# xander683/ConstructionScenePoseEstimation

Measured on AMD Instinct MI355X. Metric: annotated frames/sec (RGB+seg+2D kpts) at 1920×1080, 1/2/4/8 MI355X, higher is better.
Workload: dtype f32

## Files before the change

constructionsceneposeestimation_amd/build.py:

```python
from __future__ import annotations

import os
import shutil
import subprocess
import sys

PKG = os.path.dirname(os.path.abspath(__file__))
ROOT = os.path.dirname(PKG)
LIB = os.path.join(PKG, "libcsg.so")
SOURCES = [os.path.join(PKG, "csrc", "csg_kernels.hip"), os.path.join(PKG, "csrc", "csg_encode.hip"),
           os.path.join(PKG, "csrc", "csg_crops.hip"), os.path.join(PKG, "csrc", "csg_spans.hip"),
           os.path.join(PKG, "csrc", "csg_points.hip"), os.path.join(PKG, "csrc", "csg_amodal_spans.hip"),
           os.path.join(PKG, "csrc", "csg_mask_png.hip"), os.path.join(PKG, "csrc", "csg_jpeg.hip"),
           os.path.join(PKG, "csrc", "csg_voxels.hip"), os.path.join(PKG, "csrc", "csg_sensor.hip"),
           os.path.join(PKG, "csrc", "csg_fps.hip"),
           os.path.join(PKG, "csrc", "csg_api.cpp"), os.path.join(PKG, "csrc", "csg_passes.cpp")]
DEPS = SOURCES + [os.path.join(PKG, "csrc", "csg_ctx.h"), os.path.join(PKG, "csrc", "csg_kernels.h"), os.path.join(PKG, "csrc", "csg_encode.h"),
                  os.path.join(PKG, "csrc", "csg_deflate.h"), os.path.join(PKG, "csrc", "csg_widen.h"),
                  os.path.join(PKG, "csrc", "csg_crops.h"), os.path.join(PKG, "csrc", "csg_spans.h"),
                  os.path.join(PKG, "csrc", "csg_points.h"),
                  os.path.join(PKG, "csrc", "csg_amodal_spans.h"), os.path.join(PKG, "csrc", "csg_raster_math.h"),
                  os.path.join(PKG, "csrc", "csg_amodal_tri.inc"),
                  os.path.join(PKG, "csrc", "csg_alpha_box.h"),
                  os.path.join(PKG, "csrc", "csg_mask_png.h"), os.path.join(PKG, "csrc", "csg_bitio.h"),
                  os.path.join(PKG, "csrc", "csg_jpeg.h"), os.path.join(PKG, "csrc", "csg_voxels.h"),
                  os.path.join(PKG, "csrc", "csg_sensor.h"), os.path.join(PKG, "csrc", "csg_fps.h"),
                  os.path.join(ROOT, "include", "csg_api.h")]
ARCH = os.environ.get("CSG_OFFLOAD_ARCH", "gfx950")
IO_LIB = os.path.join(PKG, "libcsgio.so")
IO_SOURCES = [os.path.join(PKG, "csrc", "csg_io.cpp")]
IO_DEPS = IO_SOURCES + [os.path.join(ROOT, "include", "csg_io.h"), os.path.join(PKG, "csrc", "csg_repr.h")]
IO_FLAGS = ["-O3", "-std=c++17", "-fPIC", "-shared", "-Wall", "-pthread"]
JSON_EXT = os.path.join(PKG, "_csgjson.so")
JSON_SOURCES = [os.path.join(PKG, "csrc", "csg_json.cpp"), os.path.join(PKG, "csrc", "csg_repr.h")]

FLAGS = ["-O3", "-std=c++17", "-fPIC", "-shared", "-ffp-contract=off", f"--offload-arch={ARCH}", "-Wall", "-pthread"]


def hipcc() -> str:
    for c in (os.environ.get("HIPCC"), "/opt/rocm/bin/hipcc", shutil.which("hipcc")):
        if c and os.path.exists(c):
            return c
    raise RuntimeError("hipcc not found (ROCm required to build libcsg.so)")


def needs_build(lib: str = LIB, deps=None) -> bool:
    deps = DEPS if deps is None else deps
    if not os.path.exists(lib):
        return True
    t = os.path.getmtime(lib)
    return any(os.path.getmtime(p) > t for p in deps)


def build(force: bool = False, verbose: bool = False) -> str:
    if force or needs_build():
        cmd = [hipcc(), *FLAGS, "-o", LIB + ".tmp", *SOURCES]
        if verbose:
            print(" ".join(cmd), file=sys.stderr)
        subprocess.run(cmd, check=True)
        os.replace(LIB + ".tmp", LIB)
    return LIB


def build_io(force: bool = False, verbose: bool = False) -> str:
    if force or needs_build(IO_LIB, IO_DEPS):
        cxx = os.environ.get("CXX") or shutil.which("g++") or "g++"
        cmd = [cxx, *IO_FLAGS, "-o", IO_LIB + ".tmp", *IO_SOURCES, "-lz"]
        if verbose:
            print(" ".join(cmd), file=sys.stderr)
        subprocess.run(cmd, check=True)
        os.replace(IO_LIB + ".tmp", IO_LIB)
    return IO_LIB


def build_json(force: bool = False, verbose: bool = False) -> str:
    if force or needs_build(JSON_EXT, JSON_SOURCES):
        import sysconfig
        cxx = os.environ.get("CXX") or shutil.which("g++") or "g++"
        cmd = [cxx, "-O2", "-std=c++17", "-fPIC", "-shared", "-Wall", f"-I{sysconfig.get_paths()['include']}", "-o",
               JSON_EXT + ".tmp", JSON_SOURCES[0]]
        if verbose:
            print(" ".join(cmd), file=sys.stderr)
        subprocess.run(cmd, check=True)
        os.replace(JSON_EXT + ".tmp", JSON_EXT)
    return JSON_EXT


if __name__ == "__main__":
    print(build(force="--force" in sys.argv, verbose=True))
    print(build_io(force="--force" in sys.argv, verbose=True))
    print(build_json(force="--force" in sys.argv, verbose=True))
```

constructionsceneposeestimation_amd/csrc/csg_kernels.hip:

```cpp
#include <math.h>

#include <algorithm>

#include <type_traits>

#include "csg_crops.h"
#include "csg_kernels.h"
#include "csg_raster_math.h"

namespace csg {

#ifndef CSG_ABLATION
#define CSG_ABLATION 0
#endif
#define DBG(d) (CSG_ABLATION ? (d) : 0u)

constexpr uint64_t kEmptyKey = ~0ull;

__device__ __forceinline__ uint32_t fbits(float f) { return __float_as_uint(f); }

template <int Ctrl, int RowMask, int BankMask>
__device__ __forceinline__ uint32_t dpp_add(uint32_t v) {
  return v + (uint32_t)__builtin_amdgcn_update_dpp(0, (int)v, Ctrl, RowMask, BankMask, false);
}
__device__ __forceinline__ uint32_t wave_incl_scan(uint32_t v) {
  v = dpp_add<0x111, 0xf, 0xf>(v);
  v = dpp_add<0x112, 0xf, 0xf>(v);
  v = dpp_add<0x114, 0xf, 0xf>(v);
  v = dpp_add<0x118, 0xf, 0xf>(v);
  v = dpp_add<0x142, 0xa, 0xf>(v);
  v = dpp_add<0x143, 0xc, 0xf>(v);
  return v;
}

template <bool kTrail = true, int NB = kBlock>
__device__ __forceinline__ uint32_t block_excl_scan(uint32_t v, uint32_t* wsum, uint32_t& total) {
  const uint32_t inc = wave_incl_scan(v);
  const int w = threadIdx.x >> 6, lane = threadIdx.x & 63;
  if (lane == 63) wsum[w] = inc;
  __syncthreads();
  uint32_t off = 0, tot = 0;
#pragma unroll
  for (int k = 0; k < NB / 64; ++k) {
    const uint32_t x = wsum[k];
    off += (k < w) ? x : 0u;
    tot += x;
  }
  if (kTrail) __syncthreads();
  total = tot;
  return off + inc - v;
}

__device__ __forceinline__ void frame_camera(const float* V, const float* P, float* cam) {
#pragma unroll
  for (int i = 0; i < 3; ++i) {
#pragma unroll
    for (int j = 0; j < 3; ++j) cam[i * 3 + j] = V[j * 4 + i];
    cam[9 + i] = -((V[0 * 4 + i] * V[3] + V[1 * 4 + i] * V[7]) + V[2 * 4 + i] * V[11]);
  }
  cam[12] = P[0];
  cam[13] = -P[5];
  cam[14] = -P[2];
  cam[15] = -P[6];
}

__device__ __forceinline__ void unproject(const float* cam, int px, int py, float d, float out[3]) {
  const float a = ((float)px + 0.5f) - cam[14], bq = ((float)py + 0.5f) - cam[15];
  const float xc = (a * d) / cam[12], yc = -((bq * d) / cam[13]), zc = -d;
#pragma unroll
  for (int i = 0; i < 3; ++i) out[i] = ((cam[i * 3 + 0] * xc + cam[i * 3 + 1] * yc) + cam[i * 3 + 2] * zc) + cam[9 + i];
}

__device__ __forceinline__ uint32_t half_bits(float x) {
  const _Float16 h = (_Float16)(x + 0.0f);
  return (uint32_t)__builtin_bit_cast(uint16_t, h);
}

__global__ __launch_bounds__(256) void k_clip(SceneDev s, BatchDev b) {
  const uint32_t f = blockIdx.y;
  const uint32_t i = blockIdx.x * blockDim.x + threadIdx.x;
  const FrameDev& fr = b.frames[f];
  const uint32_t raw = fr.xform_set;
  const uint32_t set = raw < b.n_sets ? raw : 0u;
  if (i < s.n_inst) {
    const float* M = b.models + ((size_t)set * s.n_inst + i) * 16;
    float m[16], vm[16], c[16];
#pragma unroll
    for (int k = 0; k < 16; ++k) m[k] = M[k];
    mat4_mul(fr.view, m, vm);
    mat4_mul(fr.proj, vm, c);
    float* o = b.clip + ((size_t)f * s.n_inst + i) * 12;
#pragma unroll
    for (int k = 0; k < 4; ++k) {
      o[k] = c[k];
      o[4 + k] = c[4 + k];
      o[8 + k] = c[12 + k];
    }
  }
  if (blockIdx.x == 0 && threadIdx.x == 0) {
    b.fset[f] = set;
    if (raw >= b.n_sets) atomicOr(b.overflow, kOvBadSet);
    float pv[16];
    mat4_mul(fr.proj, fr.view, pv);
    float* o = b.pv + (size_t)f * 12;
    for (int k = 0; k < 4; ++k) {
      o[k] = pv[k];
      o[4 + k] = pv[4 + k];
      o[8 + k] = pv[12 + k];
    }
    frame_camera(fr.view, fr.proj, b.cam + (size_t)f * kCamFloats);
  }
}

__device__ __forceinline__ uint32_t rec_tile_rect(const SubRec& r, uint32_t ys) {
  const uint32_t px0 = r.g1.z & 0xFFFFu, py0 = r.g1.z >> 16, px1 = r.g1.w & 0xFFFFu, py1 = r.g1.w >> 16;
  return (px0 / kTileW) | (((py0 / kTileH) >> ys) << 8) | ((px1 / kTileW) << 16) | (((py1 / kTileH) >> ys) << 24);
}

__device__ __forceinline__ uint32_t rect_ty0(uint32_t rc, uint32_t ys) { return ((rc >> 8) & 255u) << ys; }
__device__ __forceinline__ uint32_t rect_ty1(uint32_t rc, uint32_t ys, uint32_t tiles_y) {
  return min((((rc >> 24) + 1u) << ys) - 1u, tiles_y - 1u);
}

__device__ __forceinline__ uint32_t rect_area(uint32_t rc, uint32_t ys, uint32_t tiles_y) {
  const uint32_t tx0 = rc & 255u, tx1 = (rc >> 16) & 255u;
  return (tx1 - tx0 + 1) * (rect_ty1(rc, ys, tiles_y) - rect_ty0(rc, ys) + 1);
}


__device__ __forceinline__ uint32_t rect_tile(uint32_t rc, uint32_t q, uint32_t tiles_x, uint32_t ys) {
  const uint32_t tx0 = rc & 255u, ty0 = rect_ty0(rc, ys), tx1 = (rc >> 16) & 255u;
  const uint32_t w = tx1 - tx0 + 1;
  const uint32_t r = small_div(q, w);
  return __umul24(ty0 + r, tiles_x) + tx0 + (q - __umul24(r, w));
}

typedef uint32_t v4u32 __attribute__((ext_vector_type(4)));

__device__ __forceinline__ void setup_chunk(const SceneDev& s, const BatchDev& b, const Chunk& ch, uint32_t f,
                                            int tid, int lane, uint4* sw);

__global__ __launch_bounds__(256) __attribute__((amdgpu_waves_per_eu(8, 8))) void k_setup(
    SceneDev s, BatchDev b, const Chunk* __restrict__ chunks, uint32_t n_chunks) {
  const uint32_t f = blockIdx.x, chunk = blockIdx.y + blockIdx.z * gridDim.y;
  if (chunk >= n_chunks) return;
  const int tid = threadIdx.x, lane = tid & 63;
  if (DBG(b.dbg) & 32u) return;
  const Chunk& ch = chunks[chunk];
  {
    const CullOut o = corner_out(s, ch, b.clip + ((size_t)f * s.n_inst + ch.inst) * 12, lane & 7);
    const uint64_t m8 = 0xFFull;
    const bool cull = ((__ballot(o.n) & m8) == m8) || ((__ballot(o.f) & m8) == m8) ||
                      ((__ballot(o.l) & m8) == m8) || ((__ballot(o.r) & m8) == m8) ||
                      ((__ballot(o.t) & m8) == m8) || ((__ballot(o.b) & m8) == m8);
    if (cull || (DBG(b.dbg) & 64u)) return;
  }
  static_assert(16 * kRecGroups <= 2 * 64, "two chunk stores per lane");
  __shared__ uint4 tstage[kBlock / 64][16 * kRecGroups];
  setup_chunk(s, b, ch, f, tid, lane, tstage[tid >> 6]);
}

__device__ __forceinline__ void setup_chunk(const SceneDev& s, const BatchDev& b, const Chunk& ch, uint32_t f,
                                            int tid, int lane, uint4* sw) {
  const uint32_t i = ch.inst;
  const float* Cm = b.clip + ((size_t)f * s.n_inst + i) * 12;

  SubRec r0, r1;
  uint4 c2 = make_uint4(0u, 0u, 0u, 0u), c3 = c2, c4 = c2;
  int nrec = 0;
  if ((uint32_t)tid < ch.count) {
    const uint32_t g = ch.soup + tid;
    Cv3 v[3];
    float c[12];
#pragma unroll
    for (int k = 0; k < 12; ++k) c[k] = Cm[k];
    const float* tp = s.tri_pos + (size_t)g * 9;
#pragma unroll
    for (int k = 0; k < 3; ++k) {
      const float px = tp[3 * k], py = tp[3 * k + 1], pz = tp[3 * k + 2];
      v[k].x = dot4(c + 0, px, py, pz);
      v[k].y = dot4(c + 4, px, py, pz);
      v[k].w = dot4(c + 8, px, py, pz);
    }
    const float nearc = s.near_clip, farc = s.far_clip;
    const float Wf = (float)s.W, Hf = (float)s.H;
    bool on = true, of = true, ol = true, orr = true, ot = true, ob = true;
#pragma unroll
    for (int k = 0; k < 3; ++k) {
      on &= v[k].w < nearc;
      of &= v[k].w > farc;
      ol &= v[k].x < 0.0f;
      orr &= v[k].x > Wf * v[k].w;
      ot &= v[k].y < 0.0f;
      ob &= v[k].y > Hf * v[k].w;
    }
    if ((DBG(b.dbg) & 0x10000u) && !(on | of | ol | orr | ot | ob)) {
      if (v[0].x == 1.2345e-30f && b.inst) b.inst[0] = 1;
    } else if (!(on | of | ol | orr | ot | ob)) {
      const uint32_t uid = (i << s.uid_shift) | g;
      Cv3 q0 = v[0], q1 = v[1], q2 = v[2], q3 = v[2];
      int nq = 3;
      const bool in0 = v[0].w >= nearc, in1 = v[1].w >= nearc, in2 = v[2].w >= nearc;
      if (!(in0 && in1 && in2)) {
        auto cross_pt = [&](const Cv3& a, const Cv3& bb) {
          const float tt = (nearc - a.w) / (bb.w - a.w);
          Cv3 rr;
          rr.x = a.x + tt * (bb.x - a.x);
          rr.y = a.y + tt * (bb.y - a.y);
          rr.w = nearc;
          return rr;
        };
        auto sel = [](bool c, const Cv3& a, const Cv3& bb) {
          Cv3 rr;
          rr.x = c ? a.x : bb.x;
          rr.y = c ? a.y : bb.y;
          rr.w = c ? a.w : bb.w;
          return rr;
        };
        const Cv3 I01 = cross_pt(v[0], v[1]), I12 = cross_pt(v[1], v[2]), I20 = cross_pt(v[2], v[0]);
        const int code = (int)in0 | ((int)in1 << 1) | ((int)in2 << 2);
        q0 = sel(code == 2 || code == 6, I01, sel(code == 4, I12, v[0]));
        q1 = sel(code == 1 || code == 5, I01, sel(code == 4, v[2], v[1]));
        q2 = sel(code == 1 || code == 4, I20, sel(code == 6, v[2], I12));
        q3 = sel(code == 3 || code == 6, I20, v[2]);
        nq = (code == 1 || code == 2 || code == 4) ? 3 : 4;
      }
      auto emit_tri_r = [&](const Cv3& a, float ra, const Cv3& bb, float rb, const Cv3& cc, float rc) {
        float su[3], sv[3];
        su[0] = a.x * ra; sv[0] = a.y * ra;
        su[1] = bb.x * rb; sv[1] = bb.y * rb;
        su[2] = cc.x * rc; sv[2] = cc.y * rc;
        SubRec rr;
        if (make_rec(s, su, sv, rr)) {
          if (nrec == 0) r0 = rr; else r1 = rr;
          ++nrec;
        }
      };
      auto emit_tri = [&](const Cv3& a, const Cv3& bb, const Cv3& cc) {
        emit_tri_r(a, rcp_w(a.w), bb, rcp_w(bb.w), cc, rcp_w(cc.w));
      };
      if (nq >= 3) emit_tri(q0, q1, q2);
      if (nq >= 4) emit_tri(q0, q2, q3);
      if (nrec > 0) {
        Hom h;
        hom_setup(v, h);
        if (!h.ok) {
          nrec = 0;
        } else {
          const InstSetDev is = b.iset[(size_t)b.fset[f] * s.n_inst + i];
          const uint32_t atex = is.atex == kNoAlpha ? kNoAlpha : rec_atex(is.atex, is.athr), atex_wh = is.atex_wh;
          if (is.atex != kNoAlpha && is.athr >= 255u) nrec = 0;
          float D[3], U[3] = {0.0f, 0.0f, 0.0f}, V[3] = {0.0f, 0.0f, 0.0f};
          depth_plane(h.A, h.B, h.C, h.invdet, D);
          if (is.alpha_uv) {
            const float* tu = s.tri_uv + (size_t)g * 6;
            float uv[6];
#pragma unroll
            for (int k = 0; k < 6; ++k) uv[k] = tu[k];
            uv_planes(h.A, h.B, h.C, h.invdet, uv, U, V);
            if (is.trim && nq == 3 && in0 && in1 && in2 && nrec == 1) {
              const float4 bx = s.tri_abox[g];
              const bool none = bx.x > bx.y;
              const float B = none ? 0.0f : fmaxf(fmaxf(fabsf(bx.x), fabsf(bx.y)), fmaxf(fabsf(bx.z), fabsf(bx.w)));
              float m;
              if (B < INFINITY &&
                  alpha_trim_guard(v, uv, U, V, D, (float)max(atex_wh & 0xFFFFu, atex_wh >> 16), B, m)) {
                int px0 = (int)(r0.g1.z & 0xFFFFu), py0 = (int)(r0.g1.z >> 16);
                int px1 = (int)(r0.g1.w & 0xFFFFu), py1 = (int)(r0.g1.w >> 16);
                if (none || !alpha_trim_box(U, V, D, bx, m, px0, py0, px1, py1)) {
                  nrec = 0;
                } else {
                  r0.g1.z = (uint32_t)px0 | ((uint32_t)py0 << 16);
                  r0.g1.w = (uint32_t)px1 | ((uint32_t)py1 << 16);
                }
              }
            }
          }
          c2 = make_uint4(uid, atex, __float_as_uint(D[0]), __float_as_uint(D[1]));
          c3 = make_uint4(__float_as_uint(U[0]), __float_as_uint(V[0]), __float_as_uint(U[1]), __float_as_uint(V[1]));
          c4 = make_uint4(__float_as_uint(U[2]), __float_as_uint(V[2]), __float_as_uint(D[2]), atex_wh);
        }
      }
    }
  }
  const uint64_t b1 = __ballot(nrec >= 1), b2 = __ballot(nrec >= 2);
  const uint64_t lt = (lane == 0) ? 0ull : (~0ull >> (64 - lane));
  const uint32_t mine = (uint32_t)(__popcll(b1 & lt) + __popcll(b2 & lt));
  const uint32_t wtot = (uint32_t)(__popcll(b1) + __popcll(b2));
  uint32_t wbase = 0;
  if (lane == 0 && wtot) wbase = atomicAdd(&b.rec_count[f * kCounterStride], wtot);
  wbase = __shfl(wbase, 0, 64);
  if (DBG(b.dbg) & 128u) {
    if (nrec == 3 && b.inst) b.inst[0] = r0.g0.x + r1.g0.x + c2.x + c3.x + c4.x;
    return;
  }
  const uint64_t rbase = b.slab[f].rec_base;
  const uint32_t rcap = b.slab[f].rec_cap;
  if (lane == 0 && wbase + wtot > rcap) atomicOr(b.overflow, 1u);
  uint4* dst = reinterpret_cast<uint4*>(b.recs + rbase);
  const size_t lim = (size_t)rcap * kRecGroups;
  auto put = [&](uint32_t at, const SubRec& r) {
    uint4* o = sw + at * kRecGroups;
    o[0] = r.g0;
    o[1] = r.g1;
    o[2] = c2;
    o[3] = c3;
    o[4] = c4;
  };
  for (uint32_t p0 = 0; p0 < wtot; p0 += 16) {
    if (nrec > 0 && mine - p0 < 16u) put(mine - p0, r0);
    if (nrec > 1 && mine + 1u - p0 < 16u) put(mine + 1u - p0, r1);
    __builtin_amdgcn_fence(__ATOMIC_SEQ_CST, "wavefront");
    __builtin_amdgcn_wave_barrier();
    const uint32_t nch = min(16u, wtot - p0) * kRecGroups;
    const size_t at = ((size_t)wbase + p0) * kRecGroups;
#pragma unroll
    for (uint32_t c = (uint32_t)lane; c < 2u * 64u; c += 64u)
      if (c < nch && at + c < lim) {
        const uint4 q = sw[c];
        const v4u32 w = {q.x, q.y, q.z, q.w};
        __builtin_nontemporal_store(w, reinterpret_cast<v4u32*>(dst + at + c));
      }
    __builtin_amdgcn_fence(__ATOMIC_SEQ_CST, "wavefront");
    __builtin_amdgcn_wave_barrier();
  }
  if (nrec > 0 && wbase + mine < rcap) b.rect[rbase + wbase + mine] = rec_tile_rect(r0, s.rect_ys);
  if (nrec > 1 && wbase + mine + 1 < rcap) b.rect[rbase + wbase + mine + 1] = rec_tile_rect(r1, s.rect_ys);
}

constexpr int kBinRpt = 4;
constexpr uint32_t kBinRound = kBlock * kBinRpt;
constexpr uint32_t kBinBand = 32768;

__device__ __forceinline__ int find_bin_item(const uint32_t* pre, uint32_t j) {
  int lo = 0;
#pragma unroll
  for (int step = 256; step > 0; step >>= 2) {
    const uint32_t a = pre[lo + step], b2 = pre[lo + 2 * step], c = pre[lo + 3 * step];
    lo += ((a <= j) + (b2 <= j) + (c <= j)) * step;
  }
  return lo;
}

constexpr uint32_t kCountDirect = 4;
template <uint32_t kDirect, typename Single>
__device__ __forceinline__ uint32_t bin_round_setup(const uint32_t* rect, uint32_t base, uint32_t n, uint32_t* lrc,
                                                    uint32_t* pre, uint32_t* wsum, const SceneDev& s, Single single) {
  const int tid = threadIdx.x;
  const uint32_t r0 = base + (uint32_t)tid * kBinRpt;
  uint32_t rc[kBinRpt], area[kBinRpt], sum = 0;
  static_assert(kBinRpt == 4, "one 16-B rect load per thread");
  uint4 v = make_uint4(0u, 0u, 0u, 0u);
  if (r0 + 3 < n) {
    v = *reinterpret_cast<const uint4*>(rect + r0);
  } else {
    if (r0 < n) v.x = rect[r0];
    if (r0 + 1 < n) v.y = rect[r0 + 1];
    if (r0 + 2 < n) v.z = rect[r0 + 2];
  }
  rc[0] = v.x; rc[1] = v.y; rc[2] = v.z; rc[3] = v.w;
#pragma unroll
  for (int q = 0; q < kBinRpt; ++q) {
    area[q] = (r0 + (uint32_t)q < n) ? rect_area(rc[q], s.rect_ys, s.tiles_y) : 0u;
    lrc[tid * kBinRpt + q] = rc[q];
    if (kDirect && area[q] && area[q] <= kDirect) {
#pragma clang loop unroll(disable)
      for (uint32_t a = 0; a < area[q]; ++a) single(q, rect_tile(rc[q], a, s.tiles_x, s.rect_ys));
      area[q] = 0u;
    }
  }
#pragma unroll
  for (int q = 0; q < kBinRpt; ++q) sum += area[q];
  uint32_t total;
  uint32_t ex = block_excl_scan(sum, wsum, total);
#pragma unroll
  for (int q = 0; q < kBinRpt; ++q) {
    pre[tid * kBinRpt + q] = ex;
    ex += area[q];
  }
  if (tid == kBlock - 1) pre[kBinRound] = ex;
  return total;
}

template <bool kBanded>
__global__ __launch_bounds__(256) void k_count(SceneDev s, BatchDev b) {
  extern __shared__ __attribute__((aligned(16))) uint32_t dyn_count[];
  const uint32_t band = min(s.n_tiles, kBinBand);
  uint32_t* hist = dyn_count;
  uint32_t* pre = dyn_count + ((band + 3u) & ~3u);
  uint32_t* lrc = pre + kBinRound + 4;
  uint32_t* wsum = lrc + kBinRound;
  const uint32_t f = blockIdx.y;
  const int tid = threadIdx.x;
  const uint32_t n = min(b.rec_count[f * kCounterStride], b.slab[f].rec_cap);
  const uint32_t* rect = b.rect + b.slab[f].rec_base;
  uint32_t* bc = b.bcount + ((size_t)f * gridDim.x + blockIdx.x) * s.n_tiles;
  for (uint32_t t0 = 0; t0 < s.n_tiles; t0 += band) {
    const uint32_t nb = min(band, s.n_tiles - t0);
    for (uint32_t t = tid; t < nb; t += kBlock) hist[t] = 0;
    __syncthreads();
    for (uint32_t base = blockIdx.x * kBinRound; base < n; base += gridDim.x * kBinRound) {
      const uint32_t total = bin_round_setup<kCountDirect>(rect, base, n, lrc, pre, wsum, s,
                                                   [&](int, uint32_t t) {
                                                     if (!kBanded || t - t0 < nb) atomicAdd(&hist[t - t0], 1u);
                                                   });
      __syncthreads();
      for (uint32_t j = tid; j < total; j += kBlock) {
        const int k = find_bin_item(pre, j);
        const uint32_t t = rect_tile(lrc[k], j - pre[k], s.tiles_x, s.rect_ys);
        if (!kBanded || t - t0 < nb) atomicAdd(&hist[t - t0], 1u);
      }
      __syncthreads();
    }
    for (uint32_t t = tid; t < nb; t += kBlock) bc[t0 + t] = hist[t];
    __syncthreads();
  }
}

__global__ __launch_bounds__(256) void k_colscan(SceneDev s, BatchDev b) {
  const uint32_t f = blockIdx.y, t = blockIdx.x * kBlock + threadIdx.x;
  if (t >= s.n_tiles) return;
  uint32_t* col = b.bcount + (size_t)f * b.bin_blocks * s.n_tiles + t;
  uint32_t run = 0;
#pragma unroll 8
  for (uint32_t k = 0; k < b.bin_blocks; ++k) {
    const uint32_t v = col[(size_t)k * s.n_tiles];
    col[(size_t)k * s.n_tiles] = run;
    run += v;
  }
  b.tile_count[(size_t)f * s.n_tiles + t] = run;
}

__device__ __forceinline__ uint64_t wave_incl_scan64(uint64_t v, int lane) {
#pragma unroll
  for (int o = 1; o < 64; o <<= 1) {
    const uint64_t t = __shfl_up(v, o, 64);
    if (lane >= o) v += t;
  }
  return v;
}

__global__ __launch_bounds__(64) void k_plan(const FrameDev* __restrict__ frames, uint32_t F, uint32_t def_rec,
                                             uint32_t def_bin, uint64_t rec_pool, uint64_t bin_pool, int use_hints,
                                             Slab* __restrict__ slab, uint64_t* __restrict__ need) {
  const int lane = threadIdx.x;
  uint64_t cr = 0, cb = 0;
  for (uint32_t f0 = 0; f0 < F; f0 += 64) {
    const uint32_t f = f0 + (uint32_t)lane;
    uint32_t rc = 0, bc = 0;
    if (f < F) {
      const uint32_t rh = use_hints ? frames[f].records_hint : 0u, bh = use_hints ? frames[f].bins_hint : 0u;
      rc = rh ? ((min(rh, 0x7FFFFFF0u) + 3u) & ~3u) : def_rec;
      bc = bh ? ((min(bh, 0x7FFFFFF0u) + 3u) & ~3u) : def_bin;
    }
    const uint64_t ir = wave_incl_scan64(rc, lane), ib = wave_incl_scan64(bc, lane);
    if (f < F) {
      Slab sl;
      sl.rec_base = min(cr + ir - rc, rec_pool);
      sl.bin_base = min(cb + ib - bc, bin_pool);
      sl.rec_cap = (uint32_t)min((uint64_t)rc, rec_pool - sl.rec_base);
      sl.bin_cap = (uint32_t)min((uint64_t)bc, bin_pool - sl.bin_base);
      sl.pad[0] = sl.pad[1] = 0u;
      slab[f] = sl;
    }
    cr += __shfl(ir, 63, 64);
    cb += __shfl(ib, 63, 64);
  }
  if (lane == 0) {
    need[0] = max(need[0], cr);
    need[1] = max(need[1], cb);
  }
}

__global__ __launch_bounds__(256) void k_scan(SceneDev s, BatchDev b) {
  __shared__ uint32_t wsum[kBlock / 64];
  __shared__ uint32_t carry;
  const uint32_t f = blockIdx.x;
  const uint32_t* tc = b.tile_count + (size_t)f * s.n_tiles;
  uint32_t* to = b.tile_off + (size_t)f * (s.n_tiles + 1);
  if (threadIdx.x == 0) carry = 0;
  __syncthreads();
  for (uint32_t base = 0; base < s.n_tiles; base += kBlock) {
    const uint32_t t = base + threadIdx.x;
    const uint32_t v = t < s.n_tiles ? tc[t] : 0u;
    uint32_t tot;
    const uint32_t ex = block_excl_scan(v, wsum, tot);
    const uint32_t c0 = carry;
    if (t < s.n_tiles) to[t] = c0 + ex;
    __syncthreads();
    if (threadIdx.x == 0) carry = c0 + tot;
    __syncthreads();
  }
  if (threadIdx.x == 0) {
    to[s.n_tiles] = carry;
    if (carry > b.slab[f].bin_cap) atomicOr(b.overflow, 2u);
  }
}

template <bool kBanded>
__global__ __launch_bounds__(256) void k_bin(SceneDev s, BatchDev b) {
  extern __shared__ uint32_t dyn[];
  uint32_t* hist = dyn;
  __shared__ uint32_t pre[kBinRound + 1];
  __shared__ uint32_t lrc[kBinRound];
  __shared__ uint32_t wsum[kBlock / 64];
  const uint32_t f = blockIdx.y;
  const int tid = threadIdx.x;
  const Slab sb = b.slab[f];
  const uint32_t n = min(b.rec_count[f * kCounterStride], sb.rec_cap);
  const uint32_t* rect = b.rect + sb.rec_base;
  const uint32_t* toff = b.tile_off + (size_t)f * (s.n_tiles + 1);
  uint32_t* bins = b.bins + sb.bin_base;
  const uint32_t* bo = b.bcount + ((size_t)f * gridDim.x + blockIdx.x) * s.n_tiles;
  const uint32_t* tcnt = b.tile_count + (size_t)f * s.n_tiles;
  const uint32_t band = min(s.n_tiles, kBinBand);
  for (uint32_t t0 = 0; t0 < s.n_tiles; t0 += band) {
    const uint32_t nb = min(band, s.n_tiles - t0);
    for (uint32_t t = tid; t < nb; t += kBlock)
      hist[t] = toff[t0 + t] + tcnt[t0 + t] - bo[t0 + t] - 1u;
    __syncthreads();
    for (uint32_t base = blockIdx.x * kBinRound; base < n; base += gridDim.x * kBinRound) {
      const uint32_t total = bin_round_setup<0>(rect, base, n, lrc, pre, wsum, s, [](int, uint32_t) {});
      __syncthreads();
      for (uint32_t j = tid; j < total; j += kBlock) {
        const int k = find_bin_item(pre, j);
        const uint32_t t = rect_tile(lrc[k], j - pre[k], s.tiles_x, s.rect_ys);
        if (!kBanded || t - t0 < nb) {
          const uint32_t slot = atomicSub(&hist[t - t0], 1u);
          if (slot < sb.bin_cap) bins[slot] = base + (uint32_t)k;
        }
      }
      __syncthreads();
    }
  }
}

template <bool Small>
__device__ __forceinline__ void row_span(const uint4& g0, const uint4& g1, int ox, int oy, int ly, int x0, int x1,
                                         int& xl, int& xr, bool no_exact) {
  using T = typename std::conditional<Small, int32_t, int64_t>::type;
  const int32_t RX[3] = {(int32_t)g0.x, (int32_t)g0.y, (int32_t)g0.z};
  const int32_t RY[3] = {(int32_t)g0.w, (int32_t)g1.x, (int32_t)g1.y};
  const int32_t OX = ox * 256, OY = oy * 256;
  const int32_t cy = ly * 256 + 128;
  T c0[3];
  int32_t dys[3];
  float lo = -1.0e30f, hi = 1.0e30f;
  const int ea[3] = {1, 2, 0}, eb[3] = {2, 0, 1};
#pragma unroll
  for (int e = 0; e < 3; ++e) {
    const int32_t ax = RX[ea[e]] - OX, ay = RY[ea[e]] - OY;
    const int32_t dx = RX[eb[e]] - RX[ea[e]];
    const int32_t dy = RY[eb[e]] - RY[ea[e]];
    const int bias = (dy < 0 || (dy == 0 && dx > 0)) ? 0 : -1;
    if constexpr (Small) c0[e] = __mul24(dx, cy - ay) + __mul24(dy, ax) + bias;
    else c0[e] = (int64_t)dx * (cy - ay) + (int64_t)dy * ax + bias;
    dys[e] = dy;
    const float t = (float)c0[e] * __builtin_amdgcn_rcpf((float)dy);
    hi = (dy > 0) ? fminf(hi, t) : hi;
    lo = (dy < 0) ? fmaxf(lo, t) : lo;
    hi = (dy == 0 && c0[e] < 0) ? -1.0e30f : hi;
  }
  constexpr float kEps = 1.0f / 64.0f;
  const float lc = (lo - 128.0f) * (1.0f / 256.0f), hc = (hi - 128.0f) * (1.0f / 256.0f);
  const float lcc = fminf(fmaxf(lc, (float)x0 - 1.0f), (float)x1 + 1.0f);
  const float hcc = fmaxf(fminf(hc, (float)x1 + 1.0f), (float)x0 - 1.0f);
  xl = max((int)ceilf(lcc - kEps), x0);
  xr = min((int)floorf(hcc + kEps), x1);
  const float fl = lcc - floorf(lcc), fh = hcc - floorf(hcc);
  const bool walk_l = lc > (float)x0 - 0.5f && lc < (float)x1 + 0.5f && (fl <= kEps || fl >= 1.0f - kEps);
  const bool walk_r = hc > (float)x0 - 0.5f && hc < (float)x1 + 0.5f && (fh <= kEps || fh >= 1.0f - kEps);
  if (no_exact) return;
  auto covers = [&](int lx) {
    const int32_t cx = lx * 256 + 128;
    bool in = true;
#pragma unroll
    for (int e = 0; e < 3; ++e) {
      if constexpr (Small) in &= c0[e] - __mul24(dys[e], cx) >= 0;
// ... 1531 lines not shown
```

constructionsceneposeestimation_amd/csrc/csg_raster_math.h:

```cpp
#pragma once
#include <math.h>

#include "csg_kernels.h"

namespace csg {

constexpr int kSmallCover = 4;
constexpr float kGuardPx = 1048576.0f;

typedef float f32x2 __attribute__((ext_vector_type(2)));

__device__ __forceinline__ float dot4(const float* r, float x, float y, float z) {
  return ((r[0] * x + r[1] * y) + r[2] * z) + r[3];
}

__device__ __forceinline__ void mat4_mul(const float* a, const float* b, float* c) {
#pragma unroll
  for (int i = 0; i < 4; ++i)
#pragma unroll
    for (int j = 0; j < 4; ++j)
      c[i * 4 + j] = ((a[i * 4 + 0] * b[0 * 4 + j] + a[i * 4 + 1] * b[1 * 4 + j]) + a[i * 4 + 2] * b[2 * 4 + j]) +
                     a[i * 4 + 3] * b[3 * 4 + j];
}

#ifndef CSG_FAST_RCP
#define CSG_FAST_RCP 1
#endif
__device__ __forceinline__ float rcp_ieee(float x) {
#if CSG_FAST_RCP
  const float r0 = __builtin_amdgcn_rcpf(x);
  const float e = __builtin_fmaf(-x, r0, 1.0f);
  return __builtin_fmaf(e, r0, r0);
#else
  return 1.0f / x;
#endif
}

struct Cv3 { float x, y, w; };

struct Hom {
  float A[3], B[3], C[3];
  float invdet;
  bool ok;
};

__device__ __forceinline__ void hom_setup(const Cv3* v, Hom& h) {
  const int ea[3] = {1, 2, 0}, eb[3] = {2, 0, 1};
#pragma unroll
  for (int k = 0; k < 3; ++k) {
    const Cv3 a = v[ea[k]], b = v[eb[k]];
    h.A[k] = a.y * b.w - a.w * b.y;
    h.B[k] = a.w * b.x - a.x * b.w;
    h.C[k] = a.x * b.y - a.y * b.x;
  }
  const float det = (v[0].x * h.A[0] + v[0].y * h.B[0]) + v[0].w * h.C[0];
  h.ok = det != 0.0f;
  const float ad = fabsf(det);
  h.invdet = !h.ok ? 0.0f : (ad >= 0x1p-126f && ad <= 0x1p126f) ? rcp_ieee(det) : 1.0f / det;
}

__device__ __forceinline__ void depth_plane(const float* A, const float* B, const float* C, float invdet, float* D) {
  D[0] = ((A[0] + A[1]) + A[2]) * invdet;
  D[1] = ((B[0] + B[1]) + B[2]) * invdet;
  D[2] = ((C[0] + C[1]) + C[2]) * invdet;
}
__device__ __forceinline__ void uv_planes(const float* A, const float* B, const float* C, float invdet,
                                          const float* uv, float* U, float* V) {
  U[0] = ((A[0] * uv[0] + A[1] * uv[2]) + A[2] * uv[4]) * invdet;
  U[1] = ((B[0] * uv[0] + B[1] * uv[2]) + B[2] * uv[4]) * invdet;
  U[2] = ((C[0] * uv[0] + C[1] * uv[2]) + C[2] * uv[4]) * invdet;
  V[0] = ((A[0] * uv[1] + A[1] * uv[3]) + A[2] * uv[5]) * invdet;
  V[1] = ((B[0] * uv[1] + B[1] * uv[3]) + B[2] * uv[5]) * invdet;
  V[2] = ((C[0] * uv[1] + C[1] * uv[3]) + C[2] * uv[5]) * invdet;
}

__device__ __forceinline__ float plane_at(float p0, float p1, float p2, float fx, float fy) {
  return (p0 * fx + p1 * fy) + p2;
}

struct TexTap { uint32_t i00, i10, i01, i11; int wx, wy; };

__device__ __forceinline__ int wrap_index(float fu, int n) {
  const float nf = (float)n;
  if (fu >= 0.0f && fu < nf) return (int)fu;
  const float q = floorf(fu * __builtin_amdgcn_rcpf(nf));
  float r = fu - q * nf;
  r += r < 0.0f ? nf : 0.0f;
  r -= r >= nf ? nf : 0.0f;
  return (int)r;
}

__device__ __forceinline__ f32x2 texel_coords(float u, float v, int tw, int th) {
  const f32x2 a = {u, 1.0f - v}, n = {(float)tw, (float)th};
  return a * n - 0.5f;
}

__device__ __forceinline__ TexTap tex_taps(int tw, int th, float u, float v) {
  const f32x2 t2 = texel_coords(u, v, tw, th);
  float tu = t2.x, tv = t2.y;
  if (!(fabsf(tu) < 8388608.0f)) tu = 0.0f;
  if (!(fabsf(tv) < 8388608.0f)) tv = 0.0f;
  const float fu = floorf(tu), fv = floorf(tv);
  TexTap t;
  t.wx = (int)((tu - fu) * 256.0f) & 255;
  t.wy = (int)((tv - fv) * 256.0f) & 255;
  tw &= 0x7FFF;
  const int x0 = wrap_index(fu, tw) & 0x3FFF, y0 = wrap_index(fv, th) & 0x3FFF;
  const int x1 = (x0 + 1 == tw) ? 0 : x0 + 1;
  const int y1 = (y0 + 1 == th) ? 0 : y0 + 1;
  const uint32_t r0 = __umul24((uint32_t)y0, (uint32_t)tw), r1 = __umul24((uint32_t)y1, (uint32_t)tw);
  t.i00 = r0 + (uint32_t)x0; t.i10 = r0 + (uint32_t)x1;
  t.i01 = r1 + (uint32_t)x0; t.i11 = r1 + (uint32_t)x1;
  return t;
}

__device__ __forceinline__ int bilerp8(uint32_t c00, uint32_t c10, uint32_t c01, uint32_t c11, int wx, int wy) {
  const uint32_t ax = 256u - (uint32_t)wx, ay = 256u - (uint32_t)wy;
  const uint32_t top = __umul24(c00, ax) + __umul24(c10, (uint32_t)wx);
  const uint32_t bot = __umul24(c01, ax) + __umul24(c11, (uint32_t)wx);
  return (int)((__umul24(top, ay) + __umul24(bot, (uint32_t)wy) + 32768u) >> 16);
}

__device__ __forceinline__ int div255(uint32_t x) { return (int)(__umul24(x, 32897u) >> 23); }

__device__ __forceinline__ int tex_channel(uint32_t c00, uint32_t c10, uint32_t c01, uint32_t c11, int sh, int wx,
                                           int wy) {
  return bilerp8((c00 >> sh) & 255u, (c10 >> sh) & 255u, (c01 >> sh) & 255u, (c11 >> sh) & 255u, wx, wy);
}

__device__ __forceinline__ void tex_sample(const SceneDev& s, int tid, float u, float v, int out[4]) {
  const TexDesc t = s.texd[tid];
  const TexTap k = tex_taps((int)t.width, (int)t.height, u, v);
  const uint32_t* base = reinterpret_cast<const uint32_t*>(s.texels) + t.offset;
  const uint32_t c00 = base[k.i00], c10 = base[k.i10], c01 = base[k.i01], c11 = base[k.i11];
#pragma unroll
  for (int c = 0; c < 4; ++c) out[c] = tex_channel(c00, c10, c01, c11, 8 * c, k.wx, k.wy);
}

__device__ __forceinline__ bool alpha_pass(const uint32_t* aquad, const uint32_t* acls, uint32_t offset, uint32_t wh,
                                           int thr, float u, float v) {
  const int tw = (int)(wh & 0xFFFFu), th = (int)(wh >> 16);
  const f32x2 t2 = texel_coords(u, v, tw, th);
  float tu = t2.x, tv = t2.y;
  if (!(fabsf(tu) < 8388608.0f)) tu = 0.0f;
  if (!(fabsf(tv) < 8388608.0f)) tv = 0.0f;
  const float fu = floorf(tu), fv = floorf(tv);
  const uint32_t idx = offset + __umul24((uint32_t)wrap_index(fv, th) & 0x3FFFu, (uint32_t)tw & 0x7FFFu) +
                       ((uint32_t)wrap_index(fu, tw) & 0x3FFFu);
  const uint32_t cl = (acls[idx >> 4] >> (2u * (idx & 15u))) & 3u;
  if (cl != 3u) return cl != 0u;
  const int wx = (int)((tu - fu) * 256.0f) & 255, wy = (int)((tv - fv) * 256.0f) & 255;
  const uint32_t q = aquad[idx];
  return bilerp8(q & 255u, (q >> 8) & 255u, (q >> 16) & 255u, q >> 24, wx, wy) > thr;
}

struct SubRec { uint4 g0, g1; };

__device__ __forceinline__ bool make_rec(const SceneDev& s, const float* su, const float* sv, SubRec& r) {
  int32_t x[3], y[3];
#pragma unroll
  for (int k = 0; k < 3; ++k) {
    if (!(fabsf(su[k]) < kGuardPx) || !(fabsf(sv[k]) < kGuardPx)) return false;
    x[k] = (int32_t)rintf(su[k] * 256.0f);
    y[k] = (int32_t)rintf(sv[k] * 256.0f);
  }
  const int64_t area = (int64_t)(x[1] - x[0]) * (y[2] - y[0]) - (int64_t)(x[2] - x[0]) * (y[1] - y[0]);
  if (area == 0) return false;
  if (area < 0) {
    int32_t t = x[1]; x[1] = x[2]; x[2] = t;
    t = y[1]; y[1] = y[2]; y[2] = t;
  }
  const int32_t xmin = min(x[0], min(x[1], x[2])), xmax = max(x[0], max(x[1], x[2]));
  const int32_t ymin = min(y[0], min(y[1], y[2])), ymax = max(y[0], max(y[1], y[2]));
  int px0 = (xmin - 128 + 255) >> 8, px1 = (xmax - 128) >> 8;
  int py0 = (ymin - 128 + 255) >> 8, py1 = (ymax - 128) >> 8;
  px0 = max(px0, 0);
  py0 = max(py0, 0);
  px1 = min(px1, (int)s.W - 1);
  py1 = min(py1, (int)s.H - 1);
  if (px0 > px1 || py0 > py1) return false;
  constexpr int N = kSmallCover;
  if (px1 - px0 < N && py1 - py0 < N && xmax - xmin < 8192 && ymax - ymin < 8192) {
    const int32_t cx0 = px0 * 256 + 128, cy0 = py0 * 256 + 128;
    const int ea[3] = {1, 2, 0}, eb[3] = {2, 0, 1};
    int32_t e0[3], sx[3], sy[3];
#pragma unroll
    for (int e = 0; e < 3; ++e) {
      const int32_t dx = x[eb[e]] - x[ea[e]], dy = y[eb[e]] - y[ea[e]];
      const int32_t bias = (dy < 0 || (dy == 0 && dx > 0)) ? 0 : -1;
      e0[e] = __mul24(dx, cy0 - y[ea[e]]) - __mul24(dy, cx0 - x[ea[e]]) + bias;
      sx[e] = -dy * 256;
      sy[e] = dx * 256;
    }
    const int nw = px1 - px0, nh = py1 - py0;
    uint32_t cols = 0, rows = 0;
    int nwm = 0, nhm = 0;
#pragma unroll
    for (int k = 1; k < N; ++k) {
      nwm += __any(nw >= k) ? 1 : 0;
      nhm += __any(nh >= k) ? 1 : 0;
    }
    int32_t er[3] = {e0[0], e0[1], e0[2]};
#pragma unroll
    for (int j = 0; j < N; ++j) {
      if (j > nhm) break;
      int32_t ec[3] = {er[0], er[1], er[2]};
#pragma unroll
      for (int i = 0; i < N; ++i) {
        if (i > nwm) break;
        const bool in = i <= nw && j <= nh && (ec[0] | ec[1] | ec[2]) >= 0;
        cols |= in ? 1u << i : 0u;
        rows |= in ? 1u << j : 0u;
#pragma unroll
        for (int e = 0; e < 3; ++e) ec[e] += sx[e];
      }
#pragma unroll
      for (int e = 0; e < 3; ++e) er[e] += sy[e];
    }
    if (!cols) return false;
    px1 = px0 + 31 - __clz(cols);
    px0 += __ffs(cols) - 1;
    py1 = py0 + 31 - __clz(rows);
    py0 += __ffs(rows) - 1;
  }
  r.g0 = make_uint4((uint32_t)x[0], (uint32_t)x[1], (uint32_t)x[2], (uint32_t)y[0]);
  r.g1 = make_uint4((uint32_t)y[1], (uint32_t)y[2], (uint32_t)px0 | ((uint32_t)py0 << 16),
                    (uint32_t)px1 | ((uint32_t)py1 << 16));
  return true;
}

__device__ __forceinline__ float rcp_w(float w);
constexpr float kTrimEps = 0x1p-20f;
#ifndef CSG_TRIM_PASSES
#define CSG_TRIM_PASSES 2
#endif
constexpr int kTrimPasses = CSG_TRIM_PASSES;

__device__ __forceinline__ bool alpha_trim_guard(const Cv3* v, const float* uv, const float* U, const float* V,
                                                 const float* D, float T, float B, float& m) {
  float su[3], sv[3], X = 0.0f, Y = 0.0f, umax = 0.0f;
#pragma unroll
  for (int k = 0; k < 3; ++k) {
    const float r = rcp_w(v[k].w);
    su[k] = v[k].x * r;
    sv[k] = v[k].y * r;
    X = fmaxf(X, fabsf(su[k]));
    Y = fmaxf(Y, fabsf(sv[k]));
    umax = fmaxf(umax, fmaxf(fabsf(uv[2 * k]), fabsf(uv[2 * k + 1])));
  }
  X += 1.0f;
  Y += 1.0f;
  umax += 2.0f;
  const float Sd = (fabsf(D[0]) * X + fabsf(D[1]) * Y) + fabsf(D[2]);
  const float S = fmaxf((fabsf(U[0]) * X + fabsf(U[1]) * Y) + fabsf(U[2]), (fabsf(V[0]) * X + fabsf(V[1]) * Y) + fabsf(V[2]));
  const float dD = kTrimEps * Sd + (fabsf(D[0]) + fabsf(D[1])) * (1.0f / 256.0f);
  const float dU = kTrimEps * S + fmaxf(fabsf(U[0]) + fabsf(U[1]), fabsf(V[0]) + fabsf(V[1])) * (1.0f / 256.0f);
  float dmin = INFINITY, res = 0.0f;
#pragma unroll
  for (int k = 0; k < 3; ++k) {
    const float Dk = plane_at(D[0], D[1], D[2], su[k], sv[k]);
    const float Uk = plane_at(U[0], U[1], U[2], su[k], sv[k]), Vk = plane_at(V[0], V[1], V[2], su[k], sv[k]);
    dmin = fminf(dmin, Dk);
    res = fmaxf(res, fmaxf(fabsf(Uk - uv[2 * k] * Dk), fabsf(Vk - uv[2 * k + 1] * Dk)));
  }
  dmin -= dD;
  if (!(dmin >= 0x1p-100f)) return false;
  if (!(((res + dU) + umax * dD) * T <= dmin)) return false;
  if (!(kTrimEps * T * ((S + umax * Sd) + (umax + 1.0f) * dmin) <= 0.25f * dmin)) return false;
  m = kTrimEps * (S + B * Sd);
  return m < INFINITY;
}

__device__ __forceinline__ void trim_axis(float a, float b, float c, float m, float o0, float o1, int& lo, int& hi) {
  if (!(a != 0.0f) || lo > hi) return;
  const float est = -((fmaxf(b * o0, b * o1) + c) + m) * __builtin_amdgcn_rcpf(a);
  const float e = fminf(fmaxf(est - 0.5f, (float)lo - 1.0f), (float)hi + 1.0f);
  auto gone = [&](int p) {
    const float t = (float)p + 0.5f;
    return fmaxf((a * t + b * o0) + c, (a * t + b * o1) + c) < -m;
  };
  if (a > 0.0f) {
    int n = max((int)ceilf(e), lo);
    if (n > lo && !gone(n - 1)) {
      --n;
      if (n > lo && !gone(n - 1)) n = lo;
    }
    lo = n;
  } else {
    int n = min((int)floorf(e), hi);
    if (n < hi && !gone(n + 1)) {
      ++n;
      if (n < hi && !gone(n + 1)) n = hi;
    }
    hi = n;
  }
}

__device__ __forceinline__ bool alpha_trim_box(const float* U, const float* V, const float* D, float4 bx, float m,
                                               int& px0, int& py0, int& px1, int& py1) {
#pragma nounroll
  for (int pass = 0; pass < kTrimPasses; ++pass) {
#pragma unroll
    for (int k = 0; k < 4; ++k) {
      const float* P = k < 2 ? U : V;
      const float bd = k == 0 ? bx.x : k == 1 ? bx.y : k == 2 ? bx.z : bx.w, sg = (k & 1) ? -1.0f : 1.0f;
      const float h0 = sg * (P[0] - bd * D[0]), h1 = sg * (P[1] - bd * D[1]), h2 = sg * (P[2] - bd * D[2]);
      trim_axis(h0, h1, h2, m, (float)py0 + 0.5f, (float)py1 + 0.5f, px0, px1);
      trim_axis(h1, h0, h2, m, (float)px0 + 0.5f, (float)px1 + 0.5f, py0, py1);
    }
  }
  return px0 <= px1 && py0 <= py1;
}

__device__ __forceinline__ uint32_t small_div(uint32_t q, uint32_t w) {
  uint32_t d = (uint32_t)((float)q * __builtin_amdgcn_rcpf((float)w));
  const uint32_t p = __umul24(d, w);
  d = p > q ? d - 1u : (p + w <= q ? d + 1u : d);
  return d;
}

struct CullOut { bool n, f, l, r, t, b; };
__device__ __forceinline__ CullOut corner_out(const SceneDev& s, const Chunk& ch, const float* Cm, int c) {
  const float px = (c & 4) ? ch.hi[0] : ch.lo[0];
  const float py = (c & 2) ? ch.hi[1] : ch.lo[1];
  const float pz = (c & 1) ? ch.hi[2] : ch.lo[2];
  const float X = dot4(Cm + 0, px, py, pz), Y = dot4(Cm + 4, px, py, pz), Wc = dot4(Cm + 8, px, py, pz);
  const float tol = 1e-3f * (fabsf(X) + fabsf(Y) + fabsf(Wc)) + 1e-3f;
  return CullOut{Wc < s.near_clip - tol, Wc > s.far_clip + tol, X < -tol, X > (float)s.W * Wc + tol * (float)s.W,
                 Y < -tol, Y > (float)s.H * Wc + tol * (float)s.H};
}

__device__ __forceinline__ float rcp_w(float w) { return w <= 0x1p126f ? rcp_ieee(w) : 1.0f / w; }

constexpr uint32_t kAmSerial = 16;
constexpr uint32_t kAmQueue = 64;
constexpr int32_t kAmPast = 0x7FFFFFFF;

struct AmTri {
  int32_t x[3], y[3];
  float D[3], U[3], V[3];
  uint32_t atex, wh, thr;
  uint32_t i0, ni, j0, nj;
};

template <bool kKey>
__device__ __forceinline__ bool amodal_hit(const SceneDev& s, const AmTri& t, int32_t px, int32_t py, uint32_t& key) {
  const int32_t cx = px * 256 + 128, cy = py * 256 + 128;
  const int ea[3] = {1, 2, 0}, eb[3] = {2, 0, 1};
  bool in = true;
#pragma unroll
  for (int e = 0; e < 3; ++e) {
    const int32_t dx = t.x[eb[e]] - t.x[ea[e]], dy = t.y[eb[e]] - t.y[ea[e]];
    const int32_t bias = (dy < 0 || (dy == 0 && dx > 0)) ? 0 : -1;
    in &= (int64_t)dx * (cy - t.y[ea[e]]) - (int64_t)dy * (cx - t.x[ea[e]]) + bias >= 0;
  }
  if (!in) return false;
  const float fx = (float)px + 0.5f, fy = (float)py + 0.5f;
  const float invw = plane_at(t.D[0], t.D[1], t.D[2], fx, fy);
  if (!(invw >= s.inv_far && invw <= s.inv_near)) return false;
  if constexpr (kKey) key = __float_as_uint(invw);
  if (t.atex == kNoAlpha) return true;
  const float r = rcp_ieee(invw);
  const float u = plane_at(t.U[0], t.U[1], t.U[2], fx, fy) * r, v = plane_at(t.V[0], t.V[1], t.V[2], fx, fy) * r;
  return alpha_pass(s.aquad, s.acls, t.atex, t.wh, (int)t.thr, u, v);
}

}
```

Measured before the change: 25710.

## Replace iterative alpha-box trim with triangle-clipped cut and LDS register parking

Replaces the two-pass per-axis bounding-box trimming of alpha-tested triangles with a single pass. That pass clips the triangle's vertices against each of the four alpha-box half-planes and tightens the pixel rectangle from the clipped polygon's extent. Record registers are parked in shared memory across the trim to reduce register pressure in the setup kernel. This can give tighter rectangles and fewer rasterized pixels, at the cost of extra LDS traffic and a larger shared-memory footprint per block.

```diff
diff --git a/constructionsceneposeestimation_amd/build.py b/constructionsceneposeestimation_amd/build.py
--- a/constructionsceneposeestimation_amd/build.py
+++ b/constructionsceneposeestimation_amd/build.py
@@ -21,7 +21,7 @@
                   os.path.join(PKG, "csrc", "csg_points.h"),
                   os.path.join(PKG, "csrc", "csg_amodal_spans.h"), os.path.join(PKG, "csrc", "csg_raster_math.h"),
                   os.path.join(PKG, "csrc", "csg_amodal_tri.inc"),
-                  os.path.join(PKG, "csrc", "csg_alpha_box.h"),
+                  os.path.join(PKG, "csrc", "csg_alpha_box.h"), os.path.join(PKG, "csrc", "csg_alpha_cut.h"),
                   os.path.join(PKG, "csrc", "csg_mask_png.h"), os.path.join(PKG, "csrc", "csg_bitio.h"),
                   os.path.join(PKG, "csrc", "csg_jpeg.h"), os.path.join(PKG, "csrc", "csg_voxels.h"),
                   os.path.join(PKG, "csrc", "csg_sensor.h"), os.path.join(PKG, "csrc", "csg_fps.h"),
diff --git a/constructionsceneposeestimation_amd/csrc/csg_alpha_cut.h b/constructionsceneposeestimation_amd/csrc/csg_alpha_cut.h
--- /dev/null
+++ b/constructionsceneposeestimation_amd/csrc/csg_alpha_cut.h
@@ -0,0 +1,89 @@
+#pragma once
+#include <math.h>
+#include <stdint.h>
+
+#if defined(__HIPCC__)
+#define CSG_CUT_FN __device__ __forceinline__
+#else
+#define CSG_CUT_FN inline
+#endif
+
+namespace csg {
+
+constexpr float kCutIn = 2.0f, kCutLevel = 4.0f, kCutSmall = 8.0f, kCutOuter = 12.0f;
+constexpr float kCutWiden = 0x1p-20f;
+
+CSG_CUT_FN float cut_rcp(float x) {
+#if defined(__HIPCC__)
+  return __builtin_amdgcn_rcpf(x);
+#else
+  return 1.0f / x;
+#endif
+}
+
+CSG_CUT_FN int cut_imax(int a, int b) { return a > b ? a : b; }
+CSG_CUT_FN int cut_imin(int a, int b) { return a < b ? a : b; }
+
+CSG_CUT_FN float alpha_cut_plane(int k, const float* P, const float* D, float bd, float x, float y) {
+  const float sg = (k & 1) ? -1.0f : 1.0f;
+  const float h0 = sg * (P[0] - bd * D[0]), h1 = sg * (P[1] - bd * D[1]), h2 = sg * (P[2] - bd * D[2]);
+  return (h0 * x + h1 * y) + h2;
+}
+
+CSG_CUT_FN bool alpha_cut_box(int32_t xi0, int32_t xi1, int32_t xi2, int32_t yi0, int32_t yi1, int32_t yi2,
+                              const float* U, const float* V, const float* D, float bx0, float bx1, float bx2,
+                              float bx3, float m, uint32_t& lo, uint32_t& hi) {
+  const float x0 = (float)xi0 * (1.0f / 256.0f), x1 = (float)xi1 * (1.0f / 256.0f), x2 = (float)xi2 * (1.0f / 256.0f);
+  const float y0 = (float)yi0 * (1.0f / 256.0f), y1 = (float)yi1 * (1.0f / 256.0f), y2 = (float)yi2 * (1.0f / 256.0f);
+  float xlo = -INFINITY, xhi = INFINITY, ylo = -INFINITY, yhi = INFINITY, mag = 0.0f;
+  bool any = true;
+#if defined(__HIPCC__)
+#pragma nounroll
+#endif
+  for (int k = 0; k < 4; ++k) {
+    const float sg = (k & 1) ? -1.0f : 1.0f, bd = k == 0 ? bx0 : k == 1 ? bx1 : k == 2 ? bx2 : bx3;
+    const float h0 = sg * ((k < 2 ? U[0] : V[0]) - bd * D[0]), h1 = sg * ((k < 2 ? U[1] : V[1]) - bd * D[1]);
+    const float h2 = sg * ((k < 2 ? U[2] : V[2]) - bd * D[2]);
+    const float g0 = (h0 * x0 + h1 * y0) + h2, g1 = (h0 * x1 + h1 * y1) + h2, g2 = (h0 * x2 + h1 * y2) + h2;
+    mag += (fabsf(g0) + fabsf(g1)) + fabsf(g2);
+    const bool in0 = g0 >= -kCutIn * m, in1 = g1 >= -kCutIn * m, in2 = g2 >= -kCutIn * m;
+    any = any && (in0 || in1 || in2);
+    const float rx = in0 ? x0 : in1 ? x1 : x2, ry = in0 ? y0 : in1 ? y1 : y2;
+    float nx = rx, mx = rx, ny = ry, my = ry;
+    auto point = [&](bool on, float x, float y) {
+      x = on ? x : rx;
+      y = on ? y : ry;
+      nx = fminf(nx, x); mx = fmaxf(mx, x);
+      ny = fminf(ny, y); my = fmaxf(my, y);
+    };
+    auto crossing = [&](float ga, float gb, bool ina, bool inb, float xa, float ya, float xb, float yb) {
+      const float dc = ga - gb;
+      float s = fminf(fmaxf((ga + kCutLevel * m) * cut_rcp(dc), 0.0f), 1.0f);
+      s = fabsf(dc) >= kCutSmall * m ? s : (ina ? 1.0f : 0.0f);
+      point(ina || inb, xa + s * (xb - xa), ya + s * (yb - ya));
+    };
+    point(in1, x1, y1);
+    point(in2, x2, y2);
+    crossing(g0, g1, in0, in1, x0, y0, x1, y1);
+    crossing(g1, g2, in1, in2, x1, y1, x2, y2);
+    crossing(g2, g0, in2, in0, x2, y2, x0, y0);
+    xlo = fmaxf(xlo, nx); xhi = fminf(xhi, mx);
+    ylo = fmaxf(ylo, ny); yhi = fminf(yhi, my);
+  }
+  if (!(mag < INFINITY)) return true;
+  if (!any) return false;
+  const float wx = (fmaxf(fmaxf(fabsf(x0), fabsf(x1)), fabsf(x2)) + 1.0f) * kCutWiden;
+  const float wy = (fmaxf(fmaxf(fabsf(y0), fabsf(y1)), fabsf(y2)) + 1.0f) * kCutWiden;
+  int px0 = (int)(lo & 0xFFFFu), py0 = (int)(lo >> 16), px1 = (int)(hi & 0xFFFFu), py1 = (int)(hi >> 16);
+  const float fx0 = (float)px0, fx1 = (float)px1, fy0 = (float)py0, fy1 = (float)py1;
+  px0 = cut_imax(px0, (int)ceilf(fminf(fmaxf((xlo - wx) - 0.5f, fx0 - 1.0f), fx1 + 1.0f)));
+  px1 = cut_imin(px1, (int)floorf(fminf(fmaxf((xhi + wx) - 0.5f, fx0 - 1.0f), fx1 + 1.0f)));
+  py0 = cut_imax(py0, (int)ceilf(fminf(fmaxf((ylo - wy) - 0.5f, fy0 - 1.0f), fy1 + 1.0f)));
+  py1 = cut_imin(py1, (int)floorf(fminf(fmaxf((yhi + wy) - 0.5f, fy0 - 1.0f), fy1 + 1.0f)));
+  if (px0 > px1 || py0 > py1) return false;
+  lo = (uint32_t)px0 | ((uint32_t)py0 << 16);
+  hi = (uint32_t)px1 | ((uint32_t)py1 << 16);
+  return true;
+}
+
+}
diff --git a/constructionsceneposeestimation_amd/csrc/csg_kernels.hip b/constructionsceneposeestimation_amd/csrc/csg_kernels.hip
--- a/constructionsceneposeestimation_amd/csrc/csg_kernels.hip
+++ b/constructionsceneposeestimation_amd/csrc/csg_kernels.hip
@@ -138,7 +138,7 @@
 typedef uint32_t v4u32 __attribute__((ext_vector_type(4)));
 
 __device__ __forceinline__ void setup_chunk(const SceneDev& s, const BatchDev& b, const Chunk& ch, uint32_t f,
-                                            int tid, int lane, uint4* sw);
+                                            int tid, int lane, uint4* sw, uint4* park);
 
 __global__ __launch_bounds__(256) __attribute__((amdgpu_waves_per_eu(8, 8))) void k_setup(
     SceneDev s, BatchDev b, const Chunk* __restrict__ chunks, uint32_t n_chunks) {
@@ -157,11 +157,12 @@
   }
   static_assert(16 * kRecGroups <= 2 * 64, "two chunk stores per lane");
   __shared__ uint4 tstage[kBlock / 64][16 * kRecGroups];
-  setup_chunk(s, b, ch, f, tid, lane, tstage[tid >> 6]);
+  __shared__ uint4 tpark[2][kBlock];
+  setup_chunk(s, b, ch, f, tid, lane, tstage[tid >> 6], &tpark[0][tid]);
 }
 
 __device__ __forceinline__ void setup_chunk(const SceneDev& s, const BatchDev& b, const Chunk& ch, uint32_t f,
-                                            int tid, int lane, uint4* sw) {
+                                            int tid, int lane, uint4* sw, uint4* park) {
   const uint32_t i = ch.inst;
   const float* Cm = b.clip + ((size_t)f * s.n_inst + i) * 12;
 
@@ -259,21 +260,29 @@
             for (int k = 0; k < 6; ++k) uv[k] = tu[k];
             uv_planes(h.A, h.B, h.C, h.invdet, uv, U, V);
             if (is.trim && nq == 3 && in0 && in1 && in2 && nrec == 1) {
-              const float4 bx = s.tri_abox[g];
-              const bool none = bx.x > bx.y;
-              const float B = none ? 0.0f : fmaxf(fmaxf(fabsf(bx.x), fabsf(bx.y)), fmaxf(fabsf(bx.z), fabsf(bx.w)));
+              const float4 bx0 = s.tri_abox[g];
+              const bool none = bx0.x > bx0.y;
+              const float B = none ? 0.0f : fmaxf(fmaxf(fabsf(bx0.x), fabsf(bx0.y)), fmaxf(fabsf(bx0.z), fabsf(bx0.w)));
               float m;
+              park[0] = r0.g0;
+              park[kBlock] = r0.g1;
+              asm volatile("" ::: "memory");
+              bool left = true;
               if (B < INFINITY &&
                   alpha_trim_guard(v, uv, U, V, D, (float)max(atex_wh & 0xFFFFu, atex_wh >> 16), B, m)) {
-                int px0 = (int)(r0.g1.z & 0xFFFFu), py0 = (int)(r0.g1.z >> 16);
-                int px1 = (int)(r0.g1.w & 0xFFFFu), py1 = (int)(r0.g1.w >> 16);
-                if (none || !alpha_trim_box(U, V, D, bx, m, px0, py0, px1, py1)) {
-                  nrec = 0;
-                } else {
-                  r0.g1.z = (uint32_t)px0 | ((uint32_t)py0 << 16);
-                  r0.g1.w = (uint32_t)px1 | ((uint32_t)py1 << 16);
-                }
+                asm volatile("" ::: "memory");
+                const float4 bx = s.tri_abox[g];
+                const uint4 p0 = park[0], p1 = park[kBlock];
+                uint32_t lo = p1.z, hi = p1.w;
+                left = !none && alpha_cut_box((int32_t)p0.x, (int32_t)p0.y, (int32_t)p0.z, (int32_t)p0.w, (int32_t)p1.x,
+                                              (int32_t)p1.y, U, V, D, bx.x, bx.y, bx.z, bx.w, m, lo, hi);
+                reinterpret_cast<uint32_t*>(park + kBlock)[2] = lo;
+                reinterpret_cast<uint32_t*>(park + kBlock)[3] = hi;
               }
+              asm volatile("" ::: "memory");
+              r0.g0 = park[0];
+              r0.g1 = park[kBlock];
+              if (!left) nrec = 0;
             }
           }
           c2 = make_uint4(uid, atex, __float_as_uint(D[0]), __float_as_uint(D[1]));
diff --git a/constructionsceneposeestimation_amd/csrc/csg_raster_math.h b/constructionsceneposeestimation_amd/csrc/csg_raster_math.h
--- a/constructionsceneposeestimation_amd/csrc/csg_raster_math.h
+++ b/constructionsceneposeestimation_amd/csrc/csg_raster_math.h
@@ -1,6 +1,7 @@
 #pragma once
 #include <math.h>
 
+#include "csg_alpha_cut.h"
 #include "csg_kernels.h"
 
 namespace csg {
@@ -231,10 +232,6 @@
 
 __device__ __forceinline__ float rcp_w(float w);
 constexpr float kTrimEps = 0x1p-20f;
-#ifndef CSG_TRIM_PASSES
-#define CSG_TRIM_PASSES 2
-#endif
-constexpr int kTrimPasses = CSG_TRIM_PASSES;
 
 __device__ __forceinline__ bool alpha_trim_guard(const Cv3* v, const float* uv, const float* U, const float* V,
                                                  const float* D, float T, float B, float& m) {
@@ -269,47 +266,6 @@
   if (!(kTrimEps * T * ((S + umax * Sd) + (umax + 1.0f) * dmin) <= 0.25f * dmin)) return false;
   m = kTrimEps * (S + B * Sd);
   return m < INFINITY;
-}
-
-__device__ __forceinline__ void trim_axis(float a, float b, float c, float m, float o0, float o1, int& lo, int& hi) {
-  if (!(a != 0.0f) || lo > hi) return;
-  const float est = -((fmaxf(b * o0, b * o1) + c) + m) * __builtin_amdgcn_rcpf(a);
-  const float e = fminf(fmaxf(est - 0.5f, (float)lo - 1.0f), (float)hi + 1.0f);
-  auto gone = [&](int p) {
-    const float t = (float)p + 0.5f;
-    return fmaxf((a * t + b * o0) + c, (a * t + b * o1) + c) < -m;
-  };
-  if (a > 0.0f) {
-    int n = max((int)ceilf(e), lo);
-    if (n > lo && !gone(n - 1)) {
-      --n;
-      if (n > lo && !gone(n - 1)) n = lo;
-    }
-    lo = n;
-  } else {
-    int n = min((int)floorf(e), hi);
-    if (n < hi && !gone(n + 1)) {
-      ++n;
-      if (n < hi && !gone(n + 1)) n = hi;
-    }
-    hi = n;
-  }
-}
-
-__device__ __forceinline__ bool alpha_trim_box(const float* U, const float* V, const float* D, float4 bx, float m,
-                                               int& px0, int& py0, int& px1, int& py1) {
-#pragma nounroll
-  for (int pass = 0; pass < kTrimPasses; ++pass) {
-#pragma unroll
-    for (int k = 0; k < 4; ++k) {
-      const float* P = k < 2 ? U : V;
-      const float bd = k == 0 ? bx.x : k == 1 ? bx.y : k == 2 ? bx.z : bx.w, sg = (k & 1) ? -1.0f : 1.0f;
-      const float h0 = sg * (P[0] - bd * D[0]), h1 = sg * (P[1] - bd * D[1]), h2 = sg * (P[2] - bd * D[2]);
-      trim_axis(h0, h1, h2, m, (float)py0 + 0.5f, (float)py1 + 0.5f, px0, px1);
-      trim_axis(h1, h0, h2, m, (float)px0 + 0.5f, (float)px1 + 0.5f, py0, py1);
-    }
-  }
-  return px0 <= px1 && py0 <= py1;
 }
 
 __device__ __forceinline__ uint32_t small_div(uint32_t q, uint32_t w) {
```

Result: faster. 26120 (median of 6 runs) (+1.6%).
